# mfkiwl/erlangnetwork-gnsslib-sdr

Hardware: AMD Instinct MI355X
Metric: correlations/sec (1 ms coh) + x real-time, 32-SV L1CA @16.368 Msps (higher is better)
Workload: dtype int8 samples x int8 carrier LUT -> int32 accumulators (exact); NCOs: the reference's fp64 running sums, bit for bit; 1 GPU; BASELINE configs[2]: 32-SV GPS L1CA tracking, 5-tap E/P/L correlators (CORRN=2, CORRD=3), 1 ms coherent, 16.368 Msps int8 IQ, per GPU; channels_per_gpu=32, epochs_per_launch=1000, taps=5, loop=open (frequencies held per launch); see closed_loop (--full), if_broadcast=none (1 GPU)

## Files before the change

erlangnetwork-gnsslib-sdr_amd/csrc/gnsscorr_api.hip:

```cpp
#include <cstdarg>
#include <cstdio>
#include <cstdlib>
#include <cstring>

#include "gnsscorr_ctx.h"

static thread_local char g_err[512] = "";

int gc_fail(int code, const char *fmt, ...)
{
    va_list ap;
    va_start(ap, fmt);
    vsnprintf(g_err, sizeof(g_err), fmt, ap);
    va_end(ap);
    return code;
}

int gc_fail_hip(hipError_t e, const char *what, const char *file, int line)
{
    snprintf(g_err, sizeof(g_err), "HIP error %d (%s) in %s at %s:%d", (int)e, hipGetErrorString(e), what,
             file, line);
    return GNSSCORR_EHIP;
}

extern "C" const char *gnsscorr_last_error(void) { return g_err; }

extern "C" int gnsscorr_device_count(void)
{
    int n = 0;
    if (hipGetDeviceCount(&n) != hipSuccess) return 0;
    return n;
}

static int create_handles(gnsscorr_ctx *ctx, hipStream_t stream)
{
    if (stream) ctx->stream.borrow(stream);
    else GC_TRY(ctx->stream.make());
    for (GcStream *s : {&ctx->stream_plan, &ctx->stream_finish, &ctx->stream_discover}) GC_TRY(s->make());
    for (GcEvent *ev : {&ctx->ev_spec, &ctx->ev_chain}) GC_TRY(ev->make());
    for (GcEvent *ev : {ctx->ev_plan, ctx->ev_used, ctx->ev_corr, ctx->ev_fin})
        for (int i = 0; i < 2; i++) GC_TRY(ev[i].make());
    for (GcEvent &ev : ctx->ev_burst) GC_TRY(ev.make());
    return GNSSCORR_OK;
}

extern "C" int gnsscorr_create(gnsscorr_ctx **out, int device, void *stream)
{
    if (!out) return gc_fail(GNSSCORR_EINVAL, "gnsscorr_create: null out pointer");
    int ndev = 0;
    GC_HIP(hipGetDeviceCount(&ndev));
    if (device < 0 || device >= ndev)
        return gc_fail(GNSSCORR_EHIP, "gnsscorr_create: device %d not present (%d visible)", device, ndev);
    GC_HIP(hipSetDevice(device));
    gnsscorr_ctx *ctx = new gnsscorr_ctx();
    ctx->device = device;
    int rc = create_handles(ctx, (hipStream_t)stream);
    if (rc) {
        delete ctx;
        return rc;
    }
    *out = ctx;
    return GNSSCORR_OK;
}

static void drop_channel_buffers(gnsscorr_ctx *ctx)
{
    ctx->acq = GcAcq();
    ctx->spec = GcSpec();
    ctx->dchan.reset(); ctx->dcodes.reset(); ctx->dfreqs.reset();
    ctx->state = GcTrkStateBuf();
    ctx->batch = GcBatch();
    ctx->out = GcTrkOut();
    ctx->loop = GcLoop();
    ctx->rx = GcRx();
    ctx->lock_pending = false;
}

extern "C" void gnsscorr_destroy(gnsscorr_ctx *ctx)
{
    if (!ctx) return;
    hipSetDevice(ctx->device);
    gc_quiesce(ctx, true);
    delete ctx;
}

extern "C" void *gnsscorr_stream(gnsscorr_ctx *ctx) { return ctx ? (void *)ctx->stream : nullptr; }

extern "C" int gnsscorr_sync(gnsscorr_ctx *ctx)
{
    if (!ctx) return gc_fail(GNSSCORR_EINVAL, "null context");
    GC_HIP(hipSetDevice(ctx->device));
    int rc = gc_outputs_ready(ctx);
    if (rc) return rc;
    GC_HIP(hipStreamSynchronize(ctx->stream));
    return GNSSCORR_OK;
}

static GcRing *ring_of(gnsscorr_ctx *ctx, int ftype)
{
    if (!ctx || ftype < 1 || ftype > 2) return nullptr;
    return &ctx->ring[ftype - 1];
}

static void retarget_rings(gnsscorr_ctx *ctx);

extern "C" int gnsscorr_ring_create(gnsscorr_ctx *ctx, int ftype, int dtype, uint64_t ringlen,
                                    void *devmem)
{
    GcRing *r = ring_of(ctx, ftype);
    if (!r) return gc_fail(GNSSCORR_EINVAL, "ring_create: bad context or ftype %d", ftype);
    if (dtype != 1 && dtype != 2) return gc_fail(GNSSCORR_EINVAL, "ring_create: dtype %d not 1 or 2", dtype);
    if (ringlen == 0 || ((uint64_t)dtype * ringlen) % 16 != 0)
        return gc_fail(GNSSCORR_EINVAL, "ring_create: dtype*ringlen must be a positive multiple of 16");
    if (devmem && ((uintptr_t)devmem & 15))
        return gc_fail(GNSSCORR_EINVAL, "ring_create: device buffer must be 16-byte aligned");
    GC_HIP(hipSetDevice(ctx->device));
    {
        std::lock_guard<std::mutex> lk(ctx->mtx);
        if (ctx->in.stream) GC_HIP(hipStreamSynchronize(ctx->in.stream));
        GC_HIP(hipStreamSynchronize(ctx->stream));
        r->own.reset();
        r->mem = nullptr;
        if (devmem) {
            r->mem = (int8_t *)devmem;
        } else {
            GC_RESERVE(ctx, r->own, (size_t)dtype * ringlen);
            r->mem = r->own;
            GC_HIP(hipMemsetAsync(r->mem, 0, (size_t)dtype * ringlen, ctx->stream));
            GC_HIP(hipStreamSynchronize(ctx->stream));
        }
        r->dtype = dtype;
        r->ringlen = ringlen;
        r->wrpos = 0;
    }
    retarget_rings(ctx);
    return GNSSCORR_OK;
}

#define GC_PIN_BYTES (8u << 20)

static int ingest_init(gnsscorr_ctx *ctx)
{
    GcIngest &in = ctx->in;
    if (in.ready) return GNSSCORR_OK;
    GC_TRY(in.stream.make());
    for (int i = 0; i < 2; i++) {
        GC_TRY(in.pin[i].reserve(GC_PIN_BYTES));
        GC_RESERVE(ctx, in.dstage[i], GC_PIN_BYTES);
        GC_TRY(in.ev_pin[i].make());
    }
    GC_TRY(in.ev_in.make());
    in.ready = true;
    return GNSSCORR_OK;
}

static int ingest_slot(gnsscorr_ctx *ctx, int *slot)
{
    GcIngest &in = ctx->in;
    const int s = in.pin_next;
    in.pin_next ^= 1;
    if (in.pin_busy[s]) GC_HIP(hipEventSynchronize(in.ev_pin[s]));
    in.pin_busy[s] = false;
    *slot = s;
    return GNSSCORR_OK;
}

int gc_ingest_fence(gnsscorr_ctx *ctx)
{
    if (ctx->in.in_pending) GC_HIP(hipStreamWaitEvent(ctx->stream, ctx->in.ev_in, 0));
    return GNSSCORR_OK;
}

int gc_ring_positions(gnsscorr_ctx *ctx, uint64_t wp_ring[2])
{
    std::lock_guard<std::mutex> lk(ctx->mtx);
    wp_ring[0] = ctx->ring[0].wrpos;
    wp_ring[1] = ctx->ring[1].wrpos;
    return gc_ingest_fence(ctx);
}

static int ring_write(gnsscorr_ctx *ctx, GcRing *r, uint64_t bytepos, const void *src, uint64_t bytes, hipMemcpyKind kind)
{
    const uint64_t rb = (uint64_t)r->dtype * r->ringlen;
    const uint64_t pos = bytepos % rb;
    const uint64_t first = pos + bytes <= rb ? bytes : rb - pos;
    GC_HIP(hipMemcpyAsync(r->mem + pos, src, first, kind, ctx->in.stream));
    if (first < bytes) GC_HIP(hipMemcpyAsync(r->mem, (const int8_t *)src + first, bytes - first, kind, ctx->in.stream));
    return GNSSCORR_OK;
}

extern "C" int gnsscorr_ring_push(gnsscorr_ctx *ctx, int ftype, const void *host, uint64_t nsamp)
{
    GcRing *r = ring_of(ctx, ftype);
    if (!r || !r->mem) return gc_fail(GNSSCORR_ESTATE, "ring_push: ring %d not created", ftype);
    if (nsamp > r->ringlen) return gc_fail(GNSSCORR_EINVAL, "ring_push: chunk larger than the ring");
    if (!host && nsamp) return gc_fail(GNSSCORR_EINVAL, "ring_push: null host buffer");
    GC_HIP(hipSetDevice(ctx->device));
    std::lock_guard<std::mutex> lk(ctx->mtx);
    int rc = ingest_init(ctx);
    if (rc) return rc;
    const uint64_t d = (uint64_t)r->dtype;
    const int8_t *h = (const int8_t *)host;
    uint64_t done = 0, total = d * nsamp;
    while (done < total) {
        const uint64_t piece = total - done < GC_PIN_BYTES ? total - done : GC_PIN_BYTES;
        int s;
        rc = ingest_slot(ctx, &s);
        if (rc) return rc;
        memcpy(ctx->in.pin[s], h + done, piece);
        rc = ring_write(ctx, r, d * r->wrpos + done, ctx->in.pin[s], piece, hipMemcpyHostToDevice);
        if (rc) return rc;
        GC_HIP(hipEventRecord(ctx->in.ev_pin[s], ctx->in.stream));
        ctx->in.pin_busy[s] = true;
        done += piece;
    }
    GC_HIP(hipEventRecord(ctx->in.ev_in, ctx->in.stream));
    ctx->in.in_pending = true;
    r->wrpos += nsamp;
    return GNSSCORR_OK;
}

__global__ void unpack_stereo_kernel(const uint8_t *__restrict__ src, uint64_t n, int8_t *__restrict__ r1, uint64_t len1,
                                     uint64_t pos1, int8_t *__restrict__ r2, uint64_t len2, uint64_t pos2)
{
    const uint64_t i = (uint64_t)blockIdx.x * blockDim.x + threadIdx.x;
    if (i >= n) return;
    const unsigned b = src[i];
    if (r1) r1[(pos1 + i) % len1] = (int8_t)(2 * (int)((b >> 6) & 3) - 3);
    if (r2) {
        const int vi = (b >> 3) & 7, vq = b & 7;
        const uint64_t k = (pos2 + i) % len2;
        r2[2 * k] = (int8_t)(vi < 4 ? 2 * vi + 1 : 2 * vi - 15);
        r2[2 * k + 1] = (int8_t)(vq < 4 ? 2 * vq + 1 : 2 * vq - 15);
    }
}

__global__ void unpack_rtlsdr_kernel(const uint8_t *__restrict__ src, uint64_t nbytes, int8_t *__restrict__ ring,
                                     uint64_t ringbytes, uint64_t bytepos)
{
    const uint64_t i = (uint64_t)blockIdx.x * blockDim.x + threadIdx.x;
    if (i >= nbytes) return;
    const int v = (int)src[i];
    ring[(bytepos + i) % ringbytes] = (int8_t)(v >= 128 ? v - 128 : v - 127);
}

extern "C" int gnsscorr_ring_push_packed(gnsscorr_ctx *ctx, int format, const void *host, uint64_t nsamp)
// ... 369 lines not shown
```

erlangnetwork-gnsslib-sdr_amd/csrc/gnsscorr_ctx.h:

```cpp
#pragma once

#include <map>
#include <mutex>
#include <string>
#include <type_traits>
#include <utility>
#include <vector>

#include <cstring>
#include "gnsscorr_internal.h"

struct gnsscorr_ctx;
int gc_dev_alloc(gnsscorr_ctx *ctx, void **p, size_t bytes);

template <class T>
struct GcDevBuf {
    T *p = nullptr;
    size_t n = 0;
    GcDevBuf() = default;
    GcDevBuf(GcDevBuf &&o) noexcept : p(o.p), n(o.n) { o.p = nullptr; o.n = 0; }
    GcDevBuf &operator=(GcDevBuf &&o) noexcept
    {
        if (this != &o) { reset(); p = o.p; n = o.n; o.p = nullptr; o.n = 0; }
        return *this;
// ... 5 lines not shown
        p = nullptr;
        n = 0;
    }
    int reserve(gnsscorr_ctx *ctx, size_t elems)
    {
        if (elems <= n) return 0;
        reset();
        int rc = gc_dev_alloc(ctx, (void **)&p, sizeof(T) * elems);
        if (!rc) n = elems;
        return rc;
    }
    operator T *() const { return p; }
};

template <class T>
struct GcPinBuf {
    T *p = nullptr, *dev = nullptr;
    size_t n = 0;
    GcPinBuf() = default;
    GcPinBuf(GcPinBuf &&o) noexcept : p(o.p), dev(o.dev), n(o.n) { o.p = o.dev = nullptr; o.n = 0; }
    GcPinBuf &operator=(GcPinBuf &&o) noexcept
    {
        if (this != &o) { reset(); p = o.p; dev = o.dev; n = o.n; o.p = o.dev = nullptr; o.n = 0; }
        return *this;
    }
    ~GcPinBuf() { reset(); }
    void reset()
    {
        if (p) hipHostFree(p);
        p = dev = nullptr;
        n = 0;
    }
    int reserve(size_t elems, unsigned flags = hipHostMallocDefault)
    {
        if (elems <= n) return 0;
        reset();
        GC_HIP(hipHostMalloc((void **)&p, sizeof(T) * elems, flags));
        if (flags & hipHostMallocMapped) GC_HIP(hipHostGetDevicePointer((void **)&dev, p, 0));
        n = elems;
        return 0;
    }
    operator T *() const { return p; }
};

#define GC_TRY(call)                                                            \
    do {                                                                        \
        int rc_ = (call);                                                       \
        if (rc_) return rc_;                                                    \
    } while (0)
#define GC_RESERVE(ctx, buf, elems) GC_TRY((buf).reserve((ctx), (elems)))

struct GcEvent {
    hipEvent_t e = nullptr;
    GcEvent() = default;
    GcEvent(GcEvent &&o) noexcept : e(o.e) { o.e = nullptr; }
    GcEvent &operator=(GcEvent &&o) noexcept
    {
        if (this != &o) { reset(); e = o.e; o.e = nullptr; }
        return *this;
    }
    ~GcEvent() { reset(); }
    void reset()
    {
        if (e) hipEventDestroy(e);
        e = nullptr;
    }
    int make(unsigned flags = hipEventDisableTiming)
    {
        if (!e) GC_HIP(hipEventCreateWithFlags(&e, flags));
        return 0;
    }
    operator hipEvent_t() const { return e; }
};

struct GcStream {
    hipStream_t s = nullptr;
    bool own = false;
    GcStream() = default;
    GcStream(GcStream &&o) noexcept : s(o.s), own(o.own) { o.s = nullptr; o.own = false; }
    GcStream &operator=(GcStream &&o) noexcept
    {
        if (this != &o) { reset(); s = o.s; own = o.own; o.s = nullptr; o.own = false; }
        return *this;
    }
    ~GcStream() { reset(); }
    void reset()
    {
        if (own) hipStreamDestroy(s);
        s = nullptr;
        own = false;
    }
    int make()
    {
        if (s) return 0;
        GC_HIP(hipStreamCreateWithFlags(&s, hipStreamNonBlocking));
        own = true;
        return 0;
    }
    void borrow(hipStream_t callers)
    {
        reset();
        s = callers;
    }
    operator hipStream_t() const { return s; }
};

static_assert(!std::is_copy_constructible<GcEvent>::value && !std::is_copy_assignable<GcEvent>::value, "GcEvent owns its event");
static_assert(!std::is_copy_constructible<GcStream>::value && !std::is_copy_assignable<GcStream>::value, "GcStream owns its stream");

struct GcRing {
    int8_t  *mem = nullptr;
    GcDevBuf<int8_t> own;
    int      dtype = 0;
    uint64_t ringlen = 0;
    uint64_t wrpos = 0;
};

struct GcTimer {
    std::vector<std::pair<GcEvent, GcEvent>> pending;
    double total_ms = 0.0;
    int launches = 0;
};

struct GcIngest {
    GcStream stream;
    GcPinBuf<int8_t> pin[2];
    GcDevBuf<uint8_t> dstage[2];
    GcEvent ev_pin[2];
    bool pin_busy[2] = {false, false};
    int pin_next = 0;
    GcEvent ev_in;
    bool in_pending = false;
    bool ready = false;
};

struct GcTrkStateBuf {
    GcDevBuf<GcTrkState> buf[2];
    int icur = 0;
    bool touched = true;
    GcTrkState *cur() const { return buf[icur]; }
    GcTrkState *next() const { return buf[icur ^ 1]; }
    void commit() { icur ^= 1; }
};

struct GcTrkOut {
    GcDevBuf<double> dcorrI, dcorrQ;
    GcDevBuf<double> dsumI, dsumQ;
    GcDevBuf<int> nsamp;
    GcDevBuf<int> dnco_overflow;
    GcDevBuf<int> dring_viol;
    size_t units = 0;
    int last_nepoch = 0;
    bool fin_pending = false;
    int fin_slot = 0;
};

struct GcPlanSlot {
    GcDevBuf<GcTrkPlan> plan;
    GcDevBuf<GcTrkUnit> unit;
    GcDevBuf<GcRound> rounds;
    GcDevBuf<GcUnitSegs> segs;
    GcDevBuf<int> partial;
    bool fin_pending = false;
};

struct GcBatch {
    GcPlanSlot slot[2];
    size_t units = 0;
    int nseg = 1;
    GcDevBuf<int> dspec2[2];
    GcDevBuf<unsigned short> detab;
    GcDevBuf<unsigned long long> dfinish;
    bool spec_pending = false;
    bool spec_ahead_valid = false;
    int spec_ahead_buf = 0, spec_ahead_nepoch = 0;
    int spec_last_buf = 0, spec_last_units = 0;
    const void *spec_ahead_state = nullptr;
    int plan_slot = 0;
    bool ahead_valid = false;
    int ahead_nepoch = 0;
};

#define GC_LOOP_AHEAD 3
struct GcLoop {
    GcDevBuf<gnsscorr_loop_t> dloop;
    std::vector<char> isset;
    GcDevBuf<GcStepMeta> dstep_meta;
    GcDevBuf<GcTrkUnit> dstep_unit;
    GcDevBuf<GcUnitSegs> dstep_segs;
    GcDevBuf<GcRound> dstep_rounds;
    GcDevBuf<int> dstep_partial;
    int step_nseg = 0;
    GcPinBuf<unsigned> hostflags;
    int kmax = 1;
    bool sync_hint = false;
    GcDevBuf<gnsscorr_trklog_t> dlog;
    GcDevBuf<int> dlapped;
    GcDevBuf<int> ddone;
    GcDevBuf<uint64_t> dwrpos;
    int run_nper = 0;
    int last_nper = 0;
};

struct GcRx {
    bool on = false;
    int retry_ms = 0;
    std::vector<gnsscorr_rxstat_t> st;
    std::vector<gnsscorr_lockprm_t> lockprm;
    std::vector<int> losses;
    int lock_on = 0;
    std::vector<int> lock_listed;
    GcDevBuf<gnsscorr_lockprm_t> dlockprm;
    GcDevBuf<gnsscorr_lock_t> dlock;
    GcPinBuf<int> lock_list;
    GcPinBuf<unsigned> lock_lost;
};

struct GcFftTables {
    GcDevBuf<float2> tw16k;
    GcDevBuf<float2> tw32k;
    GcDevBuf<float2> tw32p;
    GcDevBuf<float2> tw64p1;
    GcDevBuf<float2> tw64p3;
    bool ready = false;
};

struct GcAcqCar {
    int n, pad;
    int k0[GC_NCAR];
    GcCarSeg seg[GC_NCAR];
};

struct GcAcq {
    bool prepared = false;
    GcDevBuf<GcAcqCar> car;
    GcDevBuf<int> car_overflow;
    int L = 32768;
    GcDevBuf<float2> X;
    GcDevBuf<float2> C;
    GcDevBuf<GcAcqRow> rows;
    GcDevBuf<int> arrive;
    GcDevBuf<int> iters;
    GcDevBuf<gnsscorr_acqres_t> res;
    GcDevBuf<int> edge;
    GcDevBuf<double> P;
    int ngrid = 0, maxfreq = 0, maxintg = 0;
    int maxslot = 0;
    std::vector<int> grid_chan;
    GcDevBuf<int> d_grid_chan;
    GcDevBuf<uint64_t> d_grid_wrpos;
    GcDevBuf<int> d_list;
    int nplain = 0;
    std::vector<int> list, glist;
    std::vector<char> listed;
    bool ran = false;
};

struct GcSpec {
    GcDevBuf<float> psd;
    GcDevBuf<double> sum;
    GcDevBuf<unsigned> hist;
    GcDevBuf<int> maxd;
    GcDevBuf<float> win;
    int win_n = 0;
    GcDevBuf<uint64_t> loc;
    GcDevBuf<int> off;
    GcDevBuf<int8_t> stage;
    std::vector<uint64_t> hloc;
    std::vector<int> hoff;
    bool ran = false, has_hist = false;
    int nsnap = 0, nfft = 0, nloop = 0, dtype = 0;
    double f_sf = 0.0;
};

struct gnsscorr_ctx {
    int device = 0;
    GcStream stream;
    std::mutex mtx;

    GcRing ring[2];
    GcIngest in;

    int nch = 0;
    std::vector<GcChan> hchan;
    std::vector<gnsscorr_chan_t> hdesc;
    std::vector<std::vector<short>> hcode;
    std::vector<std::vector<double>> hfreq;
    std::vector<std::vector<int>> hcorrp;
    GcDevBuf<GcChan> dchan;
    GcDevBuf<int8_t> dcodes;
    GcDevBuf<double> dfreqs;
    int ntap = 0, smax_max = 0, max_n = 0;
    bool have_dtype[3] = {false, false, false};

    GcStream stream_plan;
    GcStream stream_finish;
    GcStream stream_discover;
    GcEvent ev_plan[2];
    GcEvent ev_used[2];
    GcEvent ev_corr[2];
    GcEvent ev_fin[2];
    GcEvent ev_spec, ev_chain;
    GcTrkStateBuf state;
    GcBatch batch;
    GcTrkOut out;
    GcLoop loop;
    GcEvent ev_burst[GC_LOOP_AHEAD];
    GcRx rx;
    GcEvent ev_lock;
    bool lock_pending = false;

    GcFftTables fft;
    GcAcq acq;
    GcSpec spec;

    GcDevBuf<signed char> dfec_sym;
    GcDevBuf<unsigned char> dfec_out;
    int fec_parts = 3;

    GcDevBuf<unsigned char> dlock_stage;

    int timing = 0;
    std::map<std::string, GcTimer> timers;

    int poison = -1;
};

struct GcTimed {
    gnsscorr_ctx *ctx;
    GcEvent a, b;
    const char *name;
    hipStream_t st;
    GcTimed(gnsscorr_ctx *c, const char *n, hipStream_t s = nullptr) : ctx(c), name(n), st(s ? s : c->stream)
    {
        if (!ctx->timing) return;
        if (ctx->timing == 2 && strcmp(n, "trk_corr") != 0 && strcmp(n, "acq_corr") != 0) return;
        if (a.make(hipEventDefault) || b.make(hipEventDefault)) { a.reset(); return; }
        hipEventRecord(a, st);
    }
    ~GcTimed()
    {
        if (!a) return;
        hipEventRecord(b, st);
        ctx->timers[name].pending.emplace_back(std::move(a), std::move(b));
    }
};

int gc_drain(gnsscorr_ctx *ctx);
int gc_quiesce(gnsscorr_ctx *ctx, bool ingest = false);
int gc_ensure_trk_outputs(gnsscorr_ctx *ctx, int nperiod);
int gc_outputs_ready(gnsscorr_ctx *ctx);
int gc_nco_check(gnsscorr_ctx *ctx);
int gc_acq_twiddles(gnsscorr_ctx *ctx);
int gc_ingest_fence(gnsscorr_ctx *ctx);
int gc_ring_positions(gnsscorr_ctx *ctx, uint64_t wp_ring[2]);
int gc_loop_take_state(gnsscorr_ctx *ctx);
int gc_acq_run_list(gnsscorr_ctx *ctx, const uint64_t wp_ring[2], const int *chlist, int n);
int gc_acq_handover(gnsscorr_ctx *ctx, bool quiesce);
int gc_trk_run_loop(gnsscorr_ctx *ctx, int nperiod, const uint64_t *wp_ch);
int gc_rx_lock_launch(gnsscorr_ctx *ctx, int nperiod);
```

erlangnetwork-gnsslib-sdr_amd/csrc/gnsscorr_trk.hip:

```cpp
#include <cstdlib>
#include <type_traits>


#include "gnsscorr_ctx.h"
#include "gnsscorr_ps.h"

namespace {


#define GC_EXP_LANES 64
struct ExpCarTable {
    int *k0;
    GcCarSeg *seg;
    int cap, n, overflow, prevk;
    bool lastzero, bad;
    __device__ void operator()(int k, double x, double d, int )
    {
        const GcCarSeg s = gc_carseg_make(x, d);
        const bool zero = s.fx == 0 && s.dfx == 0;
        if (n > 0 && zero && lastzero) return;
        if (n >= cap) { overflow = 1; return; }
        bad = bad || (n == 0 ? k != 0 : !(prevk < k));
        k0[n] = k;
        seg[n] = s;
// ... 544 lines not shown

template <int DTYPE, int NTAP, int NIT>
int launch_corr(hipStream_t st, const GcChan *chan, const GcTrkUnit *unit, const GcUnitSegs *segs, int *partial, int nch, int nepoch,
                int nseg, int ntap_stride, int ntap_lo, int max_n, int smax_max)
{
    constexpr int RED_BYTES = ((4 * 2 * NTAP * 4) + 15) & ~15;
    constexpr int SEGS = 256 * NIT * (16 / DTYPE);
    constexpr int RS = SEGS / 8 + 64;
    const int lds = (int)((DTYPE == 2 ? 512 : 1024) + RED_BYTES + 8 * RS * 4 + ((GC_NCAR + 4) & ~3) * 4 +
                          GC_NCAR * sizeof(GcCarSeg) + GC_NCODE * sizeof(GcCodeSeg));
    static const int ablate = getenv("GNSSCORR_TRK_ABLATE") ? atoi(getenv("GNSSCORR_TRK_ABLATE")) : 0;
    if (lds > 64 * 1024)
        GC_HIP(hipFuncSetAttribute((const void *)trk_corr_kernel<DTYPE, NTAP, NIT>,
                                   hipFuncAttributeMaxDynamicSharedMemorySize, lds));
    const long long total = 8LL * ((nepoch + 7) / 8) * nch * nseg;
    if (total > 0x7fffffffLL) return gc_fail(GNSSCORR_EINVAL, "trk_corr: batch too large (%lld workgroups)", total);
    dim3 grid((unsigned)total), block(256);
    hipLaunchKernelGGL((trk_corr_kernel<DTYPE, NTAP, NIT>), grid, block, lds, st, chan, unit, segs, partial, nch, nepoch,
                       nseg, ntap_stride, ntap_lo, max_n, ablate);
    GC_HIP(hipGetLastError());
    return 0;
}

template <int DTYPE, int NTAP>
int launch_corr_nit(hipStream_t st, const GcChan *chan, const GcTrkUnit *unit, const GcUnitSegs *segs, const GcRound *rounds, int *partial, int nch, int nepoch,
                    int nseg, int ntap_stride, int ntap_lo, int max_n, int smax_max, const unsigned short *etab)
{
    if (g_trk_algo == 1) {
        if (g_trk_nit == 1 || DTYPE == 1)
            return launch_corr_ps<DTYPE, NTAP, 1>(st, chan, unit, segs, rounds, partial, nch, nepoch, nseg, ntap_stride, ntap_lo, max_n, etab);
        return launch_corr_ps<DTYPE, NTAP, DTYPE == 1 ? 1 : 2>(st, chan, unit, segs, rounds, partial, nch, nepoch, nseg, ntap_stride, ntap_lo, max_n, etab);
    }
    switch (g_trk_nit) {
    default: return launch_corr<DTYPE, NTAP, 2>(st, chan, unit, segs, partial, nch, nepoch, nseg, ntap_stride, ntap_lo, max_n, smax_max);
    case 8: return launch_corr<DTYPE, NTAP, 8>(st, chan, unit, segs, partial, nch, nepoch, nseg, ntap_stride, ntap_lo, max_n, smax_max);
    case 4: return launch_corr<DTYPE, NTAP, 4>(st, chan, unit, segs, partial, nch, nepoch, nseg, ntap_stride, ntap_lo, max_n, smax_max);
    }
}

template <int DTYPE>
int launch_corr_taps(hipStream_t st, const GcChan *chan, const GcTrkUnit *unit, const GcUnitSegs *segs, const GcRound *rounds, int *partial, int nch, int nepoch,
                     int nseg, int ntap_stride, int ntap, int max_n, int smax_max, const unsigned short *etab)
{
#define GC_LC(N, LO) return launch_corr_nit<DTYPE, N>(st, chan, unit, segs, rounds, partial, nch, nepoch, nseg, ntap_stride, LO, max_n, smax_max, etab)
    if (ntap <= 3)  GC_LC(3, 0);
    if (ntap <= 5)  GC_LC(5, 3);
    if (ntap <= 7)  GC_LC(7, 5);
    if (ntap <= 13) GC_LC(13, 7);
    if (ntap <= 21) GC_LC(21, 13);
    GC_LC(33, 21);
#undef GC_LC
}

void trk_pick_nit()
{
    if (g_trk_nit) return;
    const char *a = getenv("GNSSCORR_TRK_ALGO");
    g_trk_algo = (a && a[0] == 'r') ? 2 : 1;
    const char *e = getenv("GNSSCORR_TRK_NIT");
    g_trk_nit = e ? atoi(e) : 2;
    if (g_trk_algo == 1) {
        if (g_trk_nit != 1 && g_trk_nit != 2) g_trk_nit = 2;
    } else {
        if (g_trk_nit != 2 && g_trk_nit != 4 && g_trk_nit != 8) g_trk_nit = 2;
    }
}

}

int gc_trk_nseg(int dtype, int max_n)
{
    trk_pick_nit();
    const int groups = (15 + max_n * dtype + 15) / 16 + 1;
    const int nit = g_trk_algo == 1 ? trk_ps_nit(dtype, g_trk_nit) : g_trk_nit;
    if (g_trk_algo == 1) {
        const int rounds = (groups + GC_PS_WLANES * nit - 1) / (GC_PS_WLANES * nit);
        return (rounds + GC_MAXR - 1) / GC_MAXR;
    }
    return (groups + 256 * nit - 1) / (256 * nit);
}

int gc_launch_trk_expand(hipStream_t st, const GcChan *chan, const GcTrkPlan *plan, GcTrkUnit *unit, GcUnitSegs *segs,
                         int *nsamp_out, int nch, int nepoch, GcRound *rounds, int nseg, int max_n, int *nco_overflow)
{
    trk_pick_nit();
    const int total = nch * nepoch;
    hipLaunchKernelGGL(trk_expand_kernel, dim3((total + 63) / 64), dim3(64), 0, st, chan, plan, unit, segs, nsamp_out,
                       nch, nepoch, g_trk_algo == 1 ? rounds : (GcRound *)nullptr, nseg, max_n, g_trk_nit, nco_overflow);
    GC_HIP(hipGetLastError());
    return 0;
}

int gc_launch_trk_corr(hipStream_t st, const GcChan *chan, const GcTrkUnit *unit, const GcUnitSegs *segs,
                       const GcRound *rounds, int *partial, int nch,
                       int nepoch, int nseg, int ntap_stride, int dtype, int ntap, int max_n, int smax_max,
                       const unsigned short *etab)
{
    trk_pick_nit();
    if (smax_max > 64) return gc_fail(GNSSCORR_EINVAL, "trk_corr: tap offset %d samples (<= 64 supported)", smax_max);
    static const bool noetab = getenv("GNSSCORR_TRK_NOEDGETAB") != nullptr;
    if (g_trk_algo != 1 || noetab) etab = nullptr;
    if (dtype == 2)
        return launch_corr_taps<2>(st, chan, unit, segs, rounds, partial, nch, nepoch, nseg, ntap_stride, ntap, max_n, smax_max, etab);
    if (dtype == 1)
        return launch_corr_taps<1>(st, chan, unit, segs, rounds, partial, nch, nepoch, nseg, ntap_stride, ntap, max_n, smax_max, etab);
    return gc_fail(GNSSCORR_EINVAL, "trk_corr: dtype %d not 1 or 2", dtype);
}

static int launch_trk_edges(hipStream_t st, const GcChan *chan, const GcTrkUnit *unit, const GcUnitSegs *segs, unsigned short *etab,
                        int nch, int nepoch)
{
    static const bool noetab = getenv("GNSSCORR_TRK_NOEDGETAB") != nullptr;
    trk_pick_nit();
    if (!etab || noetab || g_trk_algo != 1) return 0;
    hipLaunchKernelGGL(trk_edges_kernel, dim3(nch * nepoch), dim3(256), 0, st, chan, unit, segs, etab, nch, nepoch);
    GC_HIP(hipGetLastError());
    return 0;
}

__global__ void trk_ringcheck_kernel(const GcChan *__restrict__ chan, const GcTrkPlan *__restrict__ plan,
                                     const int8_t *ring0, uint64_t wrpos0, uint64_t wrpos1, int nch, int nepoch,
                                     int *__restrict__ viol)
{
    const int i = blockIdx.x * blockDim.x + threadIdx.x;
    if (i >= nch * nepoch) return;
    const int ch = i / nepoch;
    const GcTrkPlan p = plan[i];
    if (p.n <= 0) return;
    const uint64_t wp = chan[ch].ring == ring0 ? wrpos0 : wrpos1, rl = chan[ch].ringlen;
    if (p.buffloc + (uint64_t)p.n > wp || (wp > rl && p.buffloc < wp - rl)) atomicAdd(viol, 1);
}

static int launch_trk_ringcheck(hipStream_t st, const GcChan *chan, const GcTrkPlan *plan, const int8_t *ring0, uint64_t wrpos0,
                            uint64_t wrpos1, int nch, int nepoch, int *viol)
{
    const int total = nch * nepoch;
    hipLaunchKernelGGL(trk_ringcheck_kernel, dim3((total + 255) / 256), dim3(256), 0, st, chan, plan, ring0, wrpos0, wrpos1,
                       nch, nepoch, viol);
    GC_HIP(hipGetLastError());
    return 0;
}

int gc_launch_trk_finish(hipStream_t st, const int *partial, double *corrI, double *corrQ, double *sumI,
                         double *sumQ, unsigned long long *scratch, int nch, int nepoch, int nseg, int ntap)
{
    hipLaunchKernelGGL(trk_finish_kernel, dim3(nch, (nepoch + 255) / 256), dim3(256), 0, st, partial, corrI, corrQ,
                       sumI, sumQ, scratch, nepoch, nseg, ntap);
    GC_HIP(hipGetLastError());
    return 0;
}

int gc_drain(gnsscorr_ctx *ctx)
{
    for (hipStream_t s : {ctx->stream_plan.s, ctx->stream_finish.s, ctx->stream_discover.s, ctx->stream.s})
        GC_HIP(hipStreamSynchronize(s));
    ctx->out.fin_pending = false;
    for (GcPlanSlot &s : ctx->batch.slot) s.fin_pending = false;
    return GNSSCORR_OK;
}

int gc_quiesce(gnsscorr_ctx *ctx, bool ingest)
{
    if (ingest && ctx->in.stream) GC_HIP(hipStreamSynchronize(ctx->in.stream));
    GC_TRY(gc_drain(ctx));
    ctx->batch.ahead_valid = false;
    ctx->state.touched = true;
    return GNSSCORR_OK;
}

int gc_loop_take_state(gnsscorr_ctx *ctx)
{
    if (ctx->batch.ahead_valid || ctx->out.fin_pending) return gc_quiesce(ctx);
    ctx->state.touched = true;
    return GNSSCORR_OK;
}

int gc_outputs_ready(gnsscorr_ctx *ctx)
{
    if (ctx->out.fin_pending) GC_HIP(hipStreamWaitEvent(ctx->stream, ctx->ev_fin[ctx->out.fin_slot], 0));
    return GNSSCORR_OK;
}

int gc_ensure_trk_outputs(gnsscorr_ctx *ctx, int nperiod)
{
    GcTrkOut &o = ctx->out;
    const size_t units = (size_t)ctx->nch * nperiod;
    if (units <= o.units) return GNSSCORR_OK;
    GC_TRY(gc_drain(ctx));
    o.units = 0;
    GC_RESERVE(ctx, o.dcorrI, units * ctx->ntap);
    GC_RESERVE(ctx, o.dcorrQ, units * ctx->ntap);
    GC_RESERVE(ctx, o.nsamp, units);
    GC_RESERVE(ctx, o.dsumI, (size_t)ctx->nch * ctx->ntap);
    GC_RESERVE(ctx, o.dsumQ, (size_t)ctx->nch * ctx->ntap);
    for (GcDevBuf<int> *c : {&o.dnco_overflow, &o.dring_viol}) {
        if (*c) continue;
        GC_RESERVE(ctx, *c, 1);
        GC_HIP(hipMemsetAsync(*c, 0, sizeof(int), ctx->stream));
    }
    o.units = units;
    return GNSSCORR_OK;
}

static int ensure_batch_buffers(gnsscorr_ctx *ctx, int nepoch)
{
    GcBatch &b = ctx->batch;
    const size_t units = (size_t)ctx->nch * nepoch;
    if (units <= b.units) return GNSSCORR_OK;
    GC_TRY(gc_drain(ctx));
    b.ahead_valid = false;
    b.spec_ahead_valid = false;
    b.units = 0;
    b.nseg = 1;
    for (int i = 0; i < ctx->nch; i++) {
        const int s = gc_trk_nseg(ctx->hchan[i].dtype, ctx->max_n);
        if (s > b.nseg) b.nseg = s;
    }
    for (GcPlanSlot &s : b.slot) {
        GC_RESERVE(ctx, s.plan, units);
        GC_RESERVE(ctx, s.partial, units * b.nseg * 2 * ctx->ntap);
        GC_RESERVE(ctx, s.unit, units);
        GC_RESERVE(ctx, s.rounds, units * b.nseg * GC_MAXR);
        GC_RESERVE(ctx, s.segs, units);
    }
    for (int i = 0; i < 2; i++) GC_RESERVE(ctx, b.dspec2[i], gc_trk_spec_ints(units));
    GC_RESERVE(ctx, b.detab, units * GC_EDGTAB);
    GC_RESERVE(ctx, b.dfinish, (size_t)ctx->nch * GC_FINISH_SCRATCH);
    GC_HIP(hipMemsetAsync(b.dfinish, 0, sizeof(unsigned long long) * ctx->nch * GC_FINISH_SCRATCH, ctx->stream));
    b.units = units;
    return GNSSCORR_OK;
}

static int plan_into(gnsscorr_ctx *ctx, int s, int nepoch)
{
    GcBatch &b = ctx->batch;
    GcPlanSlot &sl = b.slot[s];
    hipStream_t ps = ctx->stream_plan;
    if (sl.fin_pending) GC_HIP(hipStreamWaitEvent(ps, ctx->ev_fin[s], 0));
    const GcTrkState *sin = ctx->state.cur();
    int buf;
    if (b.spec_pending) GC_HIP(hipStreamWaitEvent(ps, ctx->ev_spec, 0));
    if (b.spec_ahead_valid && !ctx->state.touched && b.spec_ahead_nepoch == nepoch && b.spec_ahead_state == (const void *)sin) {
        buf = b.spec_ahead_buf;
    } else {
        buf = 0;
        GcTimed t(ctx, "trk_spec", ps);
        GC_TRY(gc_launch_trk_spec(ps, ctx->dchan, sin, ctx->nch, nepoch, b.dspec2[buf], 0));
    }
    b.spec_ahead_valid = false;
    b.spec_pending = false;
    b.spec_last_buf = buf;
    b.spec_last_units = ctx->nch * nepoch;
    GC_HIP(hipEventRecord(ctx->ev_chain, ps));
    GC_HIP(hipStreamWaitEvent(ctx->stream_discover, ctx->ev_chain, 0));
    {
        GcTimed t(ctx, "trk_spec", ctx->stream_discover);
        GC_TRY(gc_launch_trk_spec(ctx->stream_discover, ctx->dchan, sin, ctx->nch, nepoch, b.dspec2[buf ^ 1], nepoch));
        GC_HIP(hipEventRecord(ctx->ev_spec, ctx->stream_discover));
    }
    b.spec_pending = true;
    b.spec_ahead_valid = true;
    b.spec_ahead_buf = buf ^ 1;
    b.spec_ahead_nepoch = nepoch;
    b.spec_ahead_state = (const void *)ctx->state.next();
    {
        GcTimed t(ctx, "trk_plan", ps);
        GC_TRY(gc_launch_trk_plan(ps, ctx->dchan, sin, ctx->state.next(), sl.plan, ctx->nch, nepoch, b.dspec2[buf]));
    }
    GC_HIP(hipEventRecord(ctx->ev_plan[s], ps));
    return GNSSCORR_OK;
}

static int correlate_slot(gnsscorr_ctx *ctx, int s, int nepoch, const uint64_t wr[2])
{
    GcBatch &b = ctx->batch;
    GcPlanSlot &sl = b.slot[s];
    {
        GcTimed t(ctx, "trk_expand");
        GC_TRY(gc_launch_trk_expand(ctx->stream, ctx->dchan, sl.plan, sl.unit, sl.segs, ctx->out.nsamp, ctx->nch, nepoch,
                                    sl.rounds, b.nseg, ctx->max_n, ctx->out.dnco_overflow));
    }
    GC_TRY(launch_trk_ringcheck(ctx->stream, ctx->dchan, sl.plan, (const int8_t *)ctx->ring[0].mem, wr[0], wr[1], ctx->nch,
                                nepoch, ctx->out.dring_viol));
    {
        GcTimed t(ctx, "trk_edges");
        GC_TRY(launch_trk_edges(ctx->stream, ctx->dchan, sl.unit, sl.segs, b.detab, ctx->nch, nepoch));
    }
    for (int dtype = 1; dtype <= 2; dtype++) {
        if (!ctx->have_dtype[dtype]) continue;
        GcTimed t(ctx, "trk_corr");
        GC_TRY(gc_launch_trk_corr(ctx->stream, ctx->dchan, sl.unit, sl.segs, sl.rounds, sl.partial, ctx->nch, nepoch, b.nseg,
                                  ctx->ntap, dtype, ctx->ntap, ctx->max_n, ctx->smax_max, b.detab));
    }
    GC_HIP(hipEventRecord(ctx->ev_corr[s], ctx->stream));
    return GNSSCORR_OK;
}

static int finish_slot(gnsscorr_ctx *ctx, int s, int nepoch)
{
    GcBatch &b = ctx->batch;
    GcTrkOut &o = ctx->out;
    hipStream_t fs = ctx->stream_finish;
    GC_HIP(hipStreamWaitEvent(fs, ctx->ev_corr[s], 0));
    GcTimed t(ctx, "trk_finish", fs);
    GC_TRY(gc_launch_trk_finish(fs, b.slot[s].partial, o.dcorrI, o.dcorrQ, o.dsumI, o.dsumQ, b.dfinish, ctx->nch, nepoch,
                                b.nseg, ctx->ntap));
    GC_HIP(hipEventRecord(ctx->ev_fin[s], fs));
    b.slot[s].fin_pending = true;
    o.fin_pending = true;
    o.fin_slot = s;
    return GNSSCORR_OK;
}

extern "C" int gnsscorr_trk_run(gnsscorr_ctx *ctx, int nepoch)
{
    if (!ctx || nepoch <= 0) return gc_fail(GNSSCORR_EINVAL, "trk_run: nepoch %d", nepoch);
    if (!ctx->nch) return gc_fail(GNSSCORR_ESTATE, "trk_run: no channels set");
    GC_HIP(hipSetDevice(ctx->device));
    GC_TRY(gc_ensure_trk_outputs(ctx, nepoch));
    GC_TRY(ensure_batch_buffers(ctx, nepoch));
    uint64_t wr[2];
    GC_TRY(gc_ring_positions(ctx, wr));
    GcBatch &b = ctx->batch;
    hipStream_t ps = ctx->stream_plan;
    const int cur = b.plan_slot;
    if (!(b.ahead_valid && b.ahead_nepoch == nepoch)) {
        if (b.ahead_valid) {
            GC_HIP(hipStreamSynchronize(ps));
            b.ahead_valid = false;
        }
        GC_HIP(hipEventRecord(ctx->ev_used[cur], ctx->stream));
        GC_HIP(hipStreamWaitEvent(ps, ctx->ev_used[cur], 0));
        GC_TRY(plan_into(ctx, cur, nepoch));
    }
    GC_HIP(hipStreamWaitEvent(ctx->stream, ctx->ev_plan[cur], 0));
    GC_TRY(correlate_slot(ctx, cur, nepoch, wr));
    b.ahead_valid = false;
    ctx->state.commit();
    b.plan_slot ^= 1;
    if (!ctx->state.touched) {
        GC_HIP(hipStreamWaitEvent(ps, ctx->ev_corr[b.plan_slot], 0));
        GC_TRY(plan_into(ctx, b.plan_slot, nepoch));
        b.ahead_valid = true;
        b.ahead_nepoch = nepoch;
    }
    ctx->state.touched = false;
    GC_TRY(finish_slot(ctx, cur, nepoch));
    ctx->out.last_nepoch = nepoch;
    ctx->loop.last_nper = 0;
    return GNSSCORR_OK;
}

int gc_nco_check(gnsscorr_ctx *ctx)
{
    GcTrkOut &o = ctx->out;
    int n = 0, v = 0;
    GC_HIP(hipMemcpy(&v, o.dring_viol, sizeof(int), hipMemcpyDeviceToHost));
    if (v) {
        GC_HIP(hipMemset(o.dring_viol, 0, sizeof(int)));
        return gc_fail(GNSSCORR_ESTATE, "tracking: %d (channel, period) units lay outside what the IF ring holds "
                       "(beyond the write position, or overwritten since): their sums are not the stream's", v);
    }
    GC_HIP(hipMemcpy(&n, o.dnco_overflow, sizeof(int), hipMemcpyDeviceToHost));
    if (!n) return GNSSCORR_OK;
    GC_HIP(hipMemset(o.dnco_overflow, 0, sizeof(int)));
    return gc_fail(GNSSCORR_EINVAL, "tracking: %d (channel, period) units need more NCO pieces than the tables hold "
                   "(more than two code periods per call, or a carrier crossing more than %d binades); their sums are zero",
                   n, GC_NCAR);
}

extern "C" int gnsscorr_trk_fetch(gnsscorr_ctx *ctx, double *trkII, double *trkQQ, int *nsamp_out)
{
    if (!ctx || !ctx->out.last_nepoch) return gc_fail(GNSSCORR_ESTATE, "trk_fetch: no completed trk_run");
    GC_HIP(hipSetDevice(ctx->device));
    GC_TRY(gc_outputs_ready(ctx));
    const GcTrkOut &o = ctx->out;
    const size_t units = (size_t)ctx->nch * o.last_nepoch;
    if (trkII) GC_HIP(hipMemcpyAsync(trkII, o.dcorrQ, sizeof(double) * units * ctx->ntap, hipMemcpyDeviceToHost, ctx->stream));
    if (trkQQ) GC_HIP(hipMemcpyAsync(trkQQ, o.dcorrI, sizeof(double) * units * ctx->ntap, hipMemcpyDeviceToHost, ctx->stream));
    if (nsamp_out) GC_HIP(hipMemcpyAsync(nsamp_out, o.nsamp, sizeof(int) * units, hipMemcpyDeviceToHost, ctx->stream));
    GC_HIP(hipStreamSynchronize(ctx->stream));
    return gc_nco_check(ctx);
}

extern "C" int gnsscorr_trk_fetch_sums(gnsscorr_ctx *ctx, double *sumI, double *sumQ)
{
    if (!ctx || !ctx->out.last_nepoch) return gc_fail(GNSSCORR_ESTATE, "trk_fetch_sums: no completed trk_run");
    if (ctx->loop.last_nper) return gc_fail(GNSSCORR_ESTATE, "trk_fetch_sums: the last run was closed loop (its sums are in gnsscorr_loop_get)");
    GC_HIP(hipSetDevice(ctx->device));
    GC_TRY(gc_outputs_ready(ctx));
    const size_t n = (size_t)ctx->nch * ctx->ntap;
    if (sumI) GC_HIP(hipMemcpyAsync(sumI, ctx->out.dsumQ, sizeof(double) * n, hipMemcpyDeviceToHost, ctx->stream));
    if (sumQ) GC_HIP(hipMemcpyAsync(sumQ, ctx->out.dsumI, sizeof(double) * n, hipMemcpyDeviceToHost, ctx->stream));
    GC_HIP(hipStreamSynchronize(ctx->stream));
    return GNSSCORR_OK;
}

extern "C" int gnsscorr_trk_devptrs(gnsscorr_ctx *ctx, void **trkII, void **trkQQ)
{
    if (!ctx || !ctx->out.dcorrI) return gc_fail(GNSSCORR_ESTATE, "trk_devptrs: no trk_run yet");
    GC_TRY(gc_outputs_ready(ctx));
    if (trkII) *trkII = ctx->out.dcorrQ;
    if (trkQQ) *trkQQ = ctx->out.dcorrI;
    return GNSSCORR_OK;
}

extern "C" int gnsscorr_trk_set_state(gnsscorr_ctx *ctx, int ch0, int nch, const gnsscorr_trkstate_t *st)
{
    if (!ctx || !st || ch0 < 0 || nch <= 0 || ch0 + nch > ctx->nch)
        return gc_fail(GNSSCORR_EINVAL, "trk_set_state: channel range [%d,%d) of %d", ch0, ch0 + nch, ctx ? ctx->nch : 0);
    static_assert(sizeof(gnsscorr_trkstate_t) == sizeof(GcTrkState), "state layout");
    GC_HIP(hipSetDevice(ctx->device));
    GC_TRY(gc_quiesce(ctx));
    GC_HIP(hipMemcpyAsync(ctx->state.cur() + ch0, st, sizeof(GcTrkState) * nch, hipMemcpyHostToDevice, ctx->stream));
    GC_HIP(hipStreamSynchronize(ctx->stream));
    return GNSSCORR_OK;
}

extern "C" int gnsscorr_trk_get_state(gnsscorr_ctx *ctx, int ch0, int nch, gnsscorr_trkstate_t *st)
{
    if (!ctx || !st || ch0 < 0 || nch <= 0 || ch0 + nch > ctx->nch)
        return gc_fail(GNSSCORR_EINVAL, "trk_get_state: channel range [%d,%d) of %d", ch0, ch0 + nch, ctx ? ctx->nch : 0);
    GC_HIP(hipSetDevice(ctx->device));
    GC_TRY(gc_drain(ctx));
    GC_HIP(hipMemcpyAsync(st, ctx->state.cur() + ch0, sizeof(GcTrkState) * nch, hipMemcpyDeviceToHost, ctx->stream));
    GC_HIP(hipStreamSynchronize(ctx->stream));
    return GNSSCORR_OK;
}

extern "C" int gnsscorr_debug_spec_rows(gnsscorr_ctx *ctx, int *dst, int max_ints)
{
    if (!ctx) return -1;
    const GcBatch &b = ctx->batch;
    if (!b.dspec2[b.spec_last_buf] || !b.spec_last_units) return -1;
    GC_HIP(hipSetDevice(ctx->device));
    GC_HIP(hipDeviceSynchronize());
    const size_t ints = (size_t)2 * b.spec_last_units * GC_CLAIM_ROW;
    if ((size_t)max_ints < ints) return -2;
    GC_HIP(hipMemcpy(dst, b.dspec2[b.spec_last_buf], ints * sizeof(int), hipMemcpyDeviceToHost));
    return b.spec_last_units;
}
```

Before: 306.3 million correlations/s.

## Move expand/edges tables onto a side stream and run finish on main stream

```diff
diff --git a/erlangnetwork-gnsslib-sdr_amd/csrc/gnsscorr_api.hip b/erlangnetwork-gnsslib-sdr_amd/csrc/gnsscorr_api.hip
--- a/erlangnetwork-gnsslib-sdr_amd/csrc/gnsscorr_api.hip
+++ b/erlangnetwork-gnsslib-sdr_amd/csrc/gnsscorr_api.hip
@@ -36,9 +36,9 @@
 {
     if (stream) ctx->stream.borrow(stream);
     else GC_TRY(ctx->stream.make());
-    for (GcStream *s : {&ctx->stream_plan, &ctx->stream_finish, &ctx->stream_discover}) GC_TRY(s->make());
-    for (GcEvent *ev : {&ctx->ev_spec, &ctx->ev_chain}) GC_TRY(ev->make());
-    for (GcEvent *ev : {ctx->ev_plan, ctx->ev_used, ctx->ev_corr, ctx->ev_fin})
+    for (GcStream *s : {&ctx->stream_plan, &ctx->stream_tables, &ctx->stream_discover}) GC_TRY(s->make());
+    GC_TRY(ctx->ev_spec.make());
+    for (GcEvent *ev : {ctx->ev_plan, ctx->ev_tab, ctx->ev_used, ctx->ev_corr})
         for (int i = 0; i < 2; i++) GC_TRY(ev[i].make());
     for (GcEvent &ev : ctx->ev_burst) GC_TRY(ev.make());
     return GNSSCORR_OK;
@@ -90,8 +90,6 @@
 {
     if (!ctx) return gc_fail(GNSSCORR_EINVAL, "null context");
     GC_HIP(hipSetDevice(ctx->device));
-    int rc = gc_outputs_ready(ctx);
-    if (rc) return rc;
     GC_HIP(hipStreamSynchronize(ctx->stream));
     return GNSSCORR_OK;
 }
diff --git a/erlangnetwork-gnsslib-sdr_amd/csrc/gnsscorr_ctx.h b/erlangnetwork-gnsslib-sdr_amd/csrc/gnsscorr_ctx.h
--- a/erlangnetwork-gnsslib-sdr_amd/csrc/gnsscorr_ctx.h
+++ b/erlangnetwork-gnsslib-sdr_amd/csrc/gnsscorr_ctx.h
@@ -181,7 +181,6 @@
     size_t units = 0;
     int last_nepoch = 0;
     bool fin_pending = false;
-    int fin_slot = 0;
 };
 
 struct GcPlanSlot {
@@ -190,7 +189,7 @@
     GcDevBuf<GcRound> rounds;
     GcDevBuf<GcUnitSegs> segs;
     GcDevBuf<int> partial;
-    bool fin_pending = false;
+    GcDevBuf<unsigned short> etab;
 };
 
 struct GcBatch {
@@ -198,7 +197,6 @@
     size_t units = 0;
     int nseg = 1;
     GcDevBuf<int> dspec2[2];
-    GcDevBuf<unsigned short> detab;
     GcDevBuf<unsigned long long> dfinish;
     bool spec_pending = false;
     bool spec_ahead_valid = false;
@@ -323,13 +321,13 @@
     bool have_dtype[3] = {false, false, false};
 
     GcStream stream_plan;
-    GcStream stream_finish;
+    GcStream stream_tables;
     GcStream stream_discover;
     GcEvent ev_plan[2];
+    GcEvent ev_tab[2];
     GcEvent ev_used[2];
     GcEvent ev_corr[2];
-    GcEvent ev_fin[2];
-    GcEvent ev_spec, ev_chain;
+    GcEvent ev_spec;
     GcTrkStateBuf state;
     GcBatch batch;
     GcTrkOut out;
@@ -378,7 +376,6 @@
 int gc_drain(gnsscorr_ctx *ctx);
 int gc_quiesce(gnsscorr_ctx *ctx, bool ingest = false);
 int gc_ensure_trk_outputs(gnsscorr_ctx *ctx, int nperiod);
-int gc_outputs_ready(gnsscorr_ctx *ctx);
 int gc_nco_check(gnsscorr_ctx *ctx);
 int gc_acq_twiddles(gnsscorr_ctx *ctx);
 int gc_ingest_fence(gnsscorr_ctx *ctx);
diff --git a/erlangnetwork-gnsslib-sdr_amd/csrc/gnsscorr_trk.hip b/erlangnetwork-gnsslib-sdr_amd/csrc/gnsscorr_trk.hip
--- a/erlangnetwork-gnsslib-sdr_amd/csrc/gnsscorr_trk.hip
+++ b/erlangnetwork-gnsslib-sdr_amd/csrc/gnsscorr_trk.hip
@@ -720,10 +720,9 @@
 
 int gc_drain(gnsscorr_ctx *ctx)
 {
-    for (hipStream_t s : {ctx->stream_plan.s, ctx->stream_finish.s, ctx->stream_discover.s, ctx->stream.s})
+    for (hipStream_t s : {ctx->stream_plan.s, ctx->stream_tables.s, ctx->stream_discover.s, ctx->stream.s})
         GC_HIP(hipStreamSynchronize(s));
     ctx->out.fin_pending = false;
-    for (GcPlanSlot &s : ctx->batch.slot) s.fin_pending = false;
     return GNSSCORR_OK;
 }
 
@@ -740,12 +739,6 @@
 {
     if (ctx->batch.ahead_valid || ctx->out.fin_pending) return gc_quiesce(ctx);
     ctx->state.touched = true;
-    return GNSSCORR_OK;
-}
-
-int gc_outputs_ready(gnsscorr_ctx *ctx)
-{
-    if (ctx->out.fin_pending) GC_HIP(hipStreamWaitEvent(ctx->stream, ctx->ev_fin[ctx->out.fin_slot], 0));
     return GNSSCORR_OK;
 }
 
@@ -790,21 +783,20 @@
         GC_RESERVE(ctx, s.unit, units);
         GC_RESERVE(ctx, s.rounds, units * b.nseg * GC_MAXR);
         GC_RESERVE(ctx, s.segs, units);
+        GC_RESERVE(ctx, s.etab, units * GC_EDGTAB);
     }
     for (int i = 0; i < 2; i++) GC_RESERVE(ctx, b.dspec2[i], gc_trk_spec_ints(units));
-    GC_RESERVE(ctx, b.detab, units * GC_EDGTAB);
     GC_RESERVE(ctx, b.dfinish, (size_t)ctx->nch * GC_FINISH_SCRATCH);
     GC_HIP(hipMemsetAsync(b.dfinish, 0, sizeof(unsigned long long) * ctx->nch * GC_FINISH_SCRATCH, ctx->stream));
     b.units = units;
     return GNSSCORR_OK;
 }
 
-static int plan_into(gnsscorr_ctx *ctx, int s, int nepoch)
+static int plan_into(gnsscorr_ctx *ctx, int s, int nepoch, hipEvent_t gate)
 {
     GcBatch &b = ctx->batch;
     GcPlanSlot &sl = b.slot[s];
     hipStream_t ps = ctx->stream_plan;
-    if (sl.fin_pending) GC_HIP(hipStreamWaitEvent(ps, ctx->ev_fin[s], 0));
     const GcTrkState *sin = ctx->state.cur();
     int buf;
     if (b.spec_pending) GC_HIP(hipStreamWaitEvent(ps, ctx->ev_spec, 0));
@@ -812,6 +804,7 @@
         buf = b.spec_ahead_buf;
     } else {
         buf = 0;
+        GC_HIP(hipStreamWaitEvent(ps, ctx->ev_tab[s], 0));
         GcTimed t(ctx, "trk_spec", ps);
         GC_TRY(gc_launch_trk_spec(ps, ctx->dchan, sin, ctx->nch, nepoch, b.dspec2[buf], 0));
     }
@@ -819,13 +812,13 @@
     b.spec_pending = false;
     b.spec_last_buf = buf;
     b.spec_last_units = ctx->nch * nepoch;
-    GC_HIP(hipEventRecord(ctx->ev_chain, ps));
-    GC_HIP(hipStreamWaitEvent(ctx->stream_discover, ctx->ev_chain, 0));
+    GC_HIP(hipStreamWaitEvent(ctx->stream_discover, gate, 0));
     {
         GcTimed t(ctx, "trk_spec", ctx->stream_discover);
         GC_TRY(gc_launch_trk_spec(ctx->stream_discover, ctx->dchan, sin, ctx->nch, nepoch, b.dspec2[buf ^ 1], nepoch));
-        GC_HIP(hipEventRecord(ctx->ev_spec, ctx->stream_discover));
-    }
+    }
+    GC_HIP(hipStreamWaitEvent(ctx->stream_discover, ctx->ev_tab[s ^ 1], 0));
+    GC_HIP(hipEventRecord(ctx->ev_spec, ctx->stream_discover));
     b.spec_pending = true;
     b.spec_ahead_valid = true;
     b.spec_ahead_buf = buf ^ 1;
@@ -843,22 +836,28 @@
 {
     GcBatch &b = ctx->batch;
     GcPlanSlot &sl = b.slot[s];
-    {
-        GcTimed t(ctx, "trk_expand");
-        GC_TRY(gc_launch_trk_expand(ctx->stream, ctx->dchan, sl.plan, sl.unit, sl.segs, ctx->out.nsamp, ctx->nch, nepoch,
+    hipStream_t ts = ctx->stream_tables;
+    GC_HIP(hipStreamWaitEvent(ts, ctx->ev_plan[s], 0));
+    GC_HIP(hipStreamWaitEvent(ts, ctx->ev_corr[s], 0));
+    GC_HIP(hipStreamWaitEvent(ts, ctx->ev_corr[s ^ 1], 0));
+    {
+        GcTimed t(ctx, "trk_expand", ts);
+        GC_TRY(gc_launch_trk_expand(ts, ctx->dchan, sl.plan, sl.unit, sl.segs, ctx->out.nsamp, ctx->nch, nepoch,
                                     sl.rounds, b.nseg, ctx->max_n, ctx->out.dnco_overflow));
     }
-    GC_TRY(launch_trk_ringcheck(ctx->stream, ctx->dchan, sl.plan, (const int8_t *)ctx->ring[0].mem, wr[0], wr[1], ctx->nch,
+    GC_TRY(launch_trk_ringcheck(ts, ctx->dchan, sl.plan, (const int8_t *)ctx->ring[0].mem, wr[0], wr[1], ctx->nch,
                                 nepoch, ctx->out.dring_viol));
     {
-        GcTimed t(ctx, "trk_edges");
-        GC_TRY(launch_trk_edges(ctx->stream, ctx->dchan, sl.unit, sl.segs, b.detab, ctx->nch, nepoch));
-    }
+        GcTimed t(ctx, "trk_edges", ts);
+        GC_TRY(launch_trk_edges(ts, ctx->dchan, sl.unit, sl.segs, sl.etab, ctx->nch, nepoch));
+    }
+    GC_HIP(hipEventRecord(ctx->ev_tab[s], ts));
+    GC_HIP(hipStreamWaitEvent(ctx->stream, ctx->ev_tab[s], 0));
     for (int dtype = 1; dtype <= 2; dtype++) {
         if (!ctx->have_dtype[dtype]) continue;
         GcTimed t(ctx, "trk_corr");
         GC_TRY(gc_launch_trk_corr(ctx->stream, ctx->dchan, sl.unit, sl.segs, sl.rounds, sl.partial, ctx->nch, nepoch, b.nseg,
-                                  ctx->ntap, dtype, ctx->ntap, ctx->max_n, ctx->smax_max, b.detab));
+                                  ctx->ntap, dtype, ctx->ntap, ctx->max_n, ctx->smax_max, sl.etab));
     }
     GC_HIP(hipEventRecord(ctx->ev_corr[s], ctx->stream));
     return GNSSCORR_OK;
@@ -868,15 +867,10 @@
 {
     GcBatch &b = ctx->batch;
     GcTrkOut &o = ctx->out;
-    hipStream_t fs = ctx->stream_finish;
-    GC_HIP(hipStreamWaitEvent(fs, ctx->ev_corr[s], 0));
-    GcTimed t(ctx, "trk_finish", fs);
-    GC_TRY(gc_launch_trk_finish(fs, b.slot[s].partial, o.dcorrI, o.dcorrQ, o.dsumI, o.dsumQ, b.dfinish, ctx->nch, nepoch,
-                                b.nseg, ctx->ntap));
-    GC_HIP(hipEventRecord(ctx->ev_fin[s], fs));
-    b.slot[s].fin_pending = true;
+    GcTimed t(ctx, "trk_finish");
+    GC_TRY(gc_launch_trk_finish(ctx->stream, b.slot[s].partial, o.dcorrI, o.dcorrQ, o.dsumI, o.dsumQ, b.dfinish, ctx->nch,
+                                nepoch, b.nseg, ctx->ntap));
     o.fin_pending = true;
-    o.fin_slot = s;
     return GNSSCORR_OK;
 }
 
@@ -899,16 +893,14 @@
         }
         GC_HIP(hipEventRecord(ctx->ev_used[cur], ctx->stream));
         GC_HIP(hipStreamWaitEvent(ps, ctx->ev_used[cur], 0));
-        GC_TRY(plan_into(ctx, cur, nepoch));
-    }
-    GC_HIP(hipStreamWaitEvent(ctx->stream, ctx->ev_plan[cur], 0));
+        GC_TRY(plan_into(ctx, cur, nepoch, ctx->ev_used[cur]));
+    }
     GC_TRY(correlate_slot(ctx, cur, nepoch, wr));
     b.ahead_valid = false;
     ctx->state.commit();
     b.plan_slot ^= 1;
     if (!ctx->state.touched) {
-        GC_HIP(hipStreamWaitEvent(ps, ctx->ev_corr[b.plan_slot], 0));
-        GC_TRY(plan_into(ctx, b.plan_slot, nepoch));
+        GC_TRY(plan_into(ctx, b.plan_slot, nepoch, ctx->ev_plan[cur]));
         b.ahead_valid = true;
         b.ahead_nepoch = nepoch;
     }
@@ -941,7 +933,6 @@
 {
     if (!ctx || !ctx->out.last_nepoch) return gc_fail(GNSSCORR_ESTATE, "trk_fetch: no completed trk_run");
     GC_HIP(hipSetDevice(ctx->device));
-    GC_TRY(gc_outputs_ready(ctx));
     const GcTrkOut &o = ctx->out;
     const size_t units = (size_t)ctx->nch * o.last_nepoch;
     if (trkII) GC_HIP(hipMemcpyAsync(trkII, o.dcorrQ, sizeof(double) * units * ctx->ntap, hipMemcpyDeviceToHost, ctx->stream));
@@ -956,7 +947,6 @@
     if (!ctx || !ctx->out.last_nepoch) return gc_fail(GNSSCORR_ESTATE, "trk_fetch_sums: no completed trk_run");
     if (ctx->loop.last_nper) return gc_fail(GNSSCORR_ESTATE, "trk_fetch_sums: the last run was closed loop (its sums are in gnsscorr_loop_get)");
     GC_HIP(hipSetDevice(ctx->device));
-    GC_TRY(gc_outputs_ready(ctx));
     const size_t n = (size_t)ctx->nch * ctx->ntap;
     if (sumI) GC_HIP(hipMemcpyAsync(sumI, ctx->out.dsumQ, sizeof(double) * n, hipMemcpyDeviceToHost, ctx->stream));
     if (sumQ) GC_HIP(hipMemcpyAsync(sumQ, ctx->out.dsumI, sizeof(double) * n, hipMemcpyDeviceToHost, ctx->stream));
@@ -967,7 +957,6 @@
 extern "C" int gnsscorr_trk_devptrs(gnsscorr_ctx *ctx, void **trkII, void **trkQQ)
 {
     if (!ctx || !ctx->out.dcorrI) return gc_fail(GNSSCORR_ESTATE, "trk_devptrs: no trk_run yet");
-    GC_TRY(gc_outputs_ready(ctx));
     if (trkII) *trkII = ctx->out.dcorrQ;
     if (trkQQ) *trkQQ = ctx->out.dcorrI;
     return GNSSCORR_OK;
```

Result: faster. 313.1 million correlations/s, median of 6 (+2.2%).
